# utiasASRL/mm_masking

Hardware: AMD Instinct MI355X
Metric: scan-pairs/s (mask-CNN + 10-iter dICP fwd+bwd) (higher is better)
Workload: dtype bf16; 1 GPU; BASELINE configs[2]: train_icp_weights step fwd+bwd, batch=32 per GPU, 10 dICP iters, point-to-plane Huber, dim=2; 400x3360 polar radar -> GO-CFAR + peaks + polar->Cartesian 640x640 -> U-Net (hand-written NHWC bf16 MFMA kernels, fp32 masters) -> dICP (fp32 points, fp64 normal equations) -> rot+trans+mask_pts loss -> Adam; batch_per_gpu=32, global_batch=32, scan_pts_pad=5120, map_pts=20000, map_pts_pad=20480, icp_iters=10, parallelism=dp1, scene_density=survey (SURVEY.md 8d: 3 500-5 000 valid scan points of 5 120)

## Files before the change

### mm_masking_amd/csrc/mmk_icp.hip

```cpp
#include <math.h>
#include <stdio.h>
#include <stdlib.h>

#include <algorithm>
#include <type_traits>

#include "mmk_common.h"

namespace {

constexpr int NN_THREADS = 256;
constexpr int NN_TILE = 1024;
constexpr float NN_PAD = 3.0e18f;
constexpr int ACC_THREADS = 256;
constexpr int PART_ROWS = 32;

__host__ __device__ constexpr int nacc(int dim) { return dim == 2 ? 9 : 27; }
__host__ __device__ constexpr int npose(int dim) { return dim == 2 ? 6 : 12; }

template <int DIM>
__device__ __forceinline__ void transform_point(const float *T, const float s[3], float p[DIM])
{
    if constexpr (DIM == 2) {
        p[0] = (T[0] * s[0] + T[1] * s[1]) + T[3];
        p[1] = (T[4] * s[0] + T[5] * s[1]) + T[7];
    } else {
        p[0] = ((T[0] * s[0] + T[1] * s[1]) + T[2] * s[2]) + T[3];
        p[1] = ((T[4] * s[0] + T[5] * s[1]) + T[6] * s[2]) + T[7];
        p[2] = ((T[8] * s[0] + T[9] * s[1]) + T[10] * s[2]) + T[11];
    }
}

template <int DIM>
__device__ __forceinline__ float nn_dist(float tx, float ty, float tz, const float p[DIM])
{
    float dx = tx - p[0];
    float dy = ty - p[1];
    float d = __builtin_fmaf(dy, dy, dx * dx);
    if constexpr (DIM == 3) {
        float dz = tz - p[2];
        d = __builtin_fmaf(dz, dz, d);
    }
    return d;
}

__global__ void pack_target_kernel(const float *__restrict__ tgt, int M, int cols, int dim, int Mpad,
                                   float *__restrict__ out, float *__restrict__ dec, int dec_stride)
{
    int j = blockIdx.x * blockDim.x + threadIdx.x;
    int b = blockIdx.y;
    if (j >= Mpad) return;
    for (int c = 0; c < dim; ++c) {
        float v = NN_PAD;
        if (j < M) v = tgt[((size_t)b * M + j) * cols + c];
        out[((size_t)b * dim + c) * Mpad + j] = v;
        if (dec != nullptr && j % dec_stride == 0) dec[((size_t)b * dim + c) * (Mpad / dec_stride) + j / dec_stride] = v;
    }
}

constexpr int PF_CH = 32;

__global__ __launch_bounds__(NN_THREADS) void src_zero_scan_kernel(const float *__restrict__ src, int N, int pts, int nsb,
                                                                  int32_t *__restrict__ allzero, int32_t *__restrict__ zrep)
{
    const int sb = blockIdx.x, b = blockIdx.y;
    int first = N;
    int nonzero = 0;
    for (int q = threadIdx.x; q < pts; q += blockDim.x) {
        const int i = sb * pts + q;
        if (i < N) {
            const float *sp = src + ((size_t)b * N + i) * 3;
            const bool z = sp[0] == 0.f && sp[1] == 0.f && sp[2] == 0.f;
            nonzero |= z ? 0 : 1;
            if (z && i < first) first = i;
        }
    }
    const int any = __syncthreads_or(nonzero);
#pragma unroll
    for (int off = 32; off > 0; off >>= 1) first = min(first, __shfl_down(first, off, 64));
    if ((threadIdx.x & 63) == 0 && first < N) atomicMin(&zrep[b], first);
    if (threadIdx.x == 0) allzero[(size_t)b * nsb + sb] = any ? 0 : 1;
}

__global__ void src_units_kernel(const int32_t *__restrict__ allzero, const int32_t *__restrict__ zrep, int B, int nsb, int pts,
                                 int cap, int32_t *__restrict__ ulist, int32_t *__restrict__ ucnt)
{
    const int c = threadIdx.x;
    int n = 0;
    if (c < 8)
        for (int b = c; b < B; b += 8)
            for (int sb = 0; sb < nsb; ++sb)
                if (!(allzero[(size_t)b * nsb + sb] != 0 && zrep[b] < sb * pts)) ulist[(size_t)c * cap + n++] = (b << 12) | sb;
    if (c < 8) ucnt[c] = n;
    int mx = n;
#pragma unroll
    for (int off = 4; off > 0; off >>= 1) mx = max(mx, __shfl_down(mx, off, 64));
    if (c == 0) ucnt[8] = mx;
}

typedef __attribute__((ext_vector_type(8))) __bf16 nn_bf16x8;
typedef __attribute__((ext_vector_type(16))) float nn_f32x16;
constexpr int NNM_GROUPS = 4;
constexpr int NNM_PTS = NN_THREADS / 64 * NNM_GROUPS * 32;

__device__ __forceinline__ nn_f32x16 mfma_32x32x16_bf16_c0(nn_bf16x8 a, nn_bf16x8 b)
{
    const nn_f32x16 z = {0.f, 0.f, 0.f, 0.f, 0.f, 0.f, 0.f, 0.f, 0.f, 0.f, 0.f, 0.f, 0.f, 0.f, 0.f, 0.f};
    return __builtin_amdgcn_mfma_f32_32x32x16_bf16(a, b, z, 0, 0, 0);
}
__device__ __forceinline__ void split3(float x, __bf16 &x1, __bf16 &x2, __bf16 &x3)
{
    x1 = (__bf16)x;
    const float r = x - (float)x1;
    x2 = (__bf16)r;
    x3 = (__bf16)(r - (float)x2);
}

template <int DIM>
__global__ __launch_bounds__(NN_THREADS, DIM == 2 ? 4 : 3) void nn_mfma_kernel(
    const float *__restrict__ src, const float *__restrict__ tgtp,
    const float *__restrict__ Tk, const int32_t *__restrict__ active, const int32_t *__restrict__ prev_idx,
    const int32_t *__restrict__ ulist, const int32_t *__restrict__ ucnt, int ucap, int B,
    int N, int Mpad, int nsb, int ntu, int tiles_per_unit, int total_units, float kappa,
    unsigned long long *__restrict__ packed)
{
    static_assert((DIM == 2 || DIM == 3) && NNM_GROUPS == 4, "the matrix-core filter: 16 (dim 2) or 2 x 16 (dim 3) k-slots, 4 point groups per wave");
    constexpr int KS = DIM == 2 ? 1 : 2;
    constexpr int TT = NN_TILE / KS;
    constexpr int NCH = TT / 32;
    constexpr int TPT = TT / NN_THREADS;
    __shared__ __attribute__((aligned(16))) uint4 frag[KS][NCH][64];
    __shared__ __attribute__((aligned(16))) float lt[DIM][TT];
    const int tid = threadIdx.x, lane = tid & 63, wv = tid >> 6;
    const int col = lane & 31, half = lane >> 5;
    const int ntiles = Mpad / NN_TILE;
    if (ulist != nullptr) total_units = ucnt[8] * ntu * 8;
    const float kp1 = 1.0f + kappa;

    for (int u = blockIdx.x; u < total_units; u += gridDim.x) {
        const int xcd = u & 7;
        int rest = u >> 3;
        const int tu = rest % ntu;
        rest /= ntu;
        int sb, b;
        if (ulist != nullptr) {
            if (rest >= ucnt[xcd]) continue;
            const int code = ulist[(size_t)xcd * ucap + rest];
            sb = code & 0xfff;
            b = code >> 12;
        } else {
            sb = rest % nsb;
            b = (rest / nsb) * 8 + xcd;
        }
        if (b >= B) continue;
        if (active != nullptr && active[b] == 0) continue;

        float T[16];
#pragma unroll
        for (int i = 0; i < 16; ++i) T[i] = Tk[(size_t)b * 16 + i];
        const float *tb = tgtp + (size_t)b * DIM * Mpad;

        float px[NNM_GROUPS], py[NNM_GROUPS], pz[NNM_GROUPS], c2[NNM_GROUPS], brun[NNM_GROUPS], thr[NNM_GROUPS], dseed[NNM_GROUPS];
        int jseed[NNM_GROUPS];
        nn_bf16x8 bfr[KS][NNM_GROUPS];
        unsigned w[NNM_GROUPS];
#pragma unroll
        for (int g = 0; g < NNM_GROUPS; ++g) {
            const int i = sb * NNM_PTS + wv * (NNM_GROUPS * 32) + g * 32 + col;
            float s0 = 0.f, s1 = 0.f, s2 = 0.f;
            if (i < N) {
                const float *sp = src + ((size_t)b * N + i) * 3;
                s0 = sp[0];
                s1 = sp[1];
                s2 = sp[2];
            }
            const float s[3] = {s0, s1, s2};
            float tp[DIM];
            transform_point<DIM>(T, s, tp);
            px[g] = tp[0];
            py[g] = tp[1];
            pz[g] = DIM == 3 ? tp[DIM - 1] : 0.f;
            float pn = tp[0] * tp[0] + tp[1] * tp[1];
            if constexpr (DIM == 3) pn += tp[DIM - 1] * tp[DIM - 1];
            c2[g] = 2.0f * kappa * pn + 1e-30f;
            const float ax = -2.0f * tp[0], ay = -2.0f * tp[1], az = -2.0f * pz[g];
            __bf16 ax1, ax2, ax3, ay1, ay2, ay3;
            split3(ax, ax1, ax2, ax3);
            split3(ay, ay1, ay2, ay3);
            const __bf16 one = (__bf16)1.0f, zero = (__bf16)0.0f;
            const nn_bf16x8 lo = {ax1, ax1, ax2, ax1, ax2, ax3, ay1, ay1};
            if constexpr (DIM == 2) {
                const nn_bf16x8 hi = {ay2, ay1, ay2, ay3, one, one, one, zero};
                bfr[0][g] = half ? hi : lo;
            } else {
                __bf16 az1, az2, az3;
                split3(az, az1, az2, az3);
                const nn_bf16x8 hi = {ay2, ay1, ay2, ay3, az1, az1, az2, az1};
                const nn_bf16x8 lo1 = {az2, az3, one, one, one, zero, zero, zero};
                const nn_bf16x8 hi1 = {zero, zero, zero, zero, zero, zero, zero, zero};
                bfr[0][g] = half ? hi : lo;
                bfr[KS - 1][g] = half ? hi1 : lo1;
// ... 64 lines not shown
                    *reinterpret_cast<float2 *>(&lt[0][lpos]) = vx;
                    *reinterpret_cast<float2 *>(&lt[1][lpos]) = vy;
                    *reinterpret_cast<float2 *>(&lt[DIM - 1][lpos]) = vz;
                    xs[0] = vx.x; xs[TPT - 1] = vx.y;
                    ys[0] = vy.x; ys[TPT - 1] = vy.y;
                    zs[0] = vz.x; zs[TPT - 1] = vz.y;
                }
                uint4 *fr = &frag[0][ch][p4];
#pragma unroll
                for (int r = 0; r < TPT; ++r) {
                    float n = __builtin_fmaf(ys[r], ys[r], xs[r] * xs[r]);
                    if constexpr (DIM == 3) n = __builtin_fmaf(zs[r], zs[r], n);
                    __bf16 x1, x2, x3, y1, y2, y3, n1, n2, n3;
                    split3(xs[r], x1, x2, x3);
                    split3(ys[r], y1, y2, y3);
                    split3(n, n1, n2, n3);
                    const nn_bf16x8 lo = {x1, x2, x1, x3, x2, x1, y1, y2};
                    fr[r] = __builtin_bit_cast(uint4, lo);
                    if constexpr (DIM == 2) {
                        const nn_bf16x8 hi = {y1, y3, y2, y1, n1, n2, n3, (__bf16)0.0f};
                        fr[32 + r] = __builtin_bit_cast(uint4, hi);
                    } else {
                        __bf16 z1, z2, z3;
                        split3(zs[r], z1, z2, z3);
                        const __bf16 zero = (__bf16)0.0f;
                        const nn_bf16x8 hi = {y1, y3, y2, y1, z1, z2, z1, z3};
                        const nn_bf16x8 lo1 = {z2, z1, n1, n2, n3, zero, zero, zero};
                        const nn_bf16x8 hi1 = {zero, zero, zero, zero, zero, zero, zero, zero};
                        fr[32 + r] = __builtin_bit_cast(uint4, hi);
                        uint4 *fr1 = &frag[KS - 1][ch][p4];
                        fr1[r] = __builtin_bit_cast(uint4, lo1);
                        fr1[32 + r] = __builtin_bit_cast(uint4, hi1);
                    }
                }
            }
            __syncthreads();
#pragma unroll
            for (int g = 0; g < NNM_GROUPS; ++g) w[g] = 0u;
            auto reduce = [&](const nn_f32x16 &acc, int g, bool refresh) {
                auto m3 = [](float a, float b, float c) { return __builtin_fminf(__builtin_fminf(a, b), c); };
                const float m0 = m3(thr[g], acc[0], acc[1]), m1 = m3(acc[2], acc[3], acc[4]), m2 = m3(acc[5], acc[6], acc[7]);
                const float m4 = m3(acc[8], acc[9], acc[10]), m5 = m3(acc[11], acc[12], acc[13]);
                const float n0 = m3(m0, m1, m2), n1 = m3(m4, m5, acc[14]);
                const float t = m3(n0, n1, acc[15]);
                w[g] = __builtin_amdgcn_alignbit(w[g], __float_as_uint(t - thr[g]), 31);
                brun[g] = __builtin_fminf(brun[g], t);
                if (refresh) thr[g] = __builtin_fmaf(brun[g], kp1, c2[g]);
            };
            uint4 af_next[KS];
#pragma unroll
            for (int k = 0; k < KS; ++k) af_next[k] = frag[k][0][lane];
#pragma unroll 2
            for (int c = 0; c < NCH; ++c) {
                nn_bf16x8 af[KS];
#pragma unroll
                for (int k = 0; k < KS; ++k) {
                    af[k] = __builtin_bit_cast(nn_bf16x8, af_next[k]);
                    af_next[k] = frag[k][(c + 1) & (NCH - 1)][lane];
                }
                const bool refresh = (c & 1) != 0;
#pragma unroll
                for (int h2 = 0; h2 < NNM_GROUPS; h2 += 2) {
                    nn_f32x16 acc0 = mfma_32x32x16_bf16_c0(af[0], bfr[0][h2]);
                    nn_f32x16 acc1 = mfma_32x32x16_bf16_c0(af[0], bfr[0][h2 + 1]);
                    if constexpr (KS == 2) {
                        acc0 = __builtin_amdgcn_mfma_f32_32x32x16_bf16(af[KS - 1], bfr[KS - 1][h2], acc0, 0, 0, 0);
                        acc1 = __builtin_amdgcn_mfma_f32_32x32x16_bf16(af[KS - 1], bfr[KS - 1][h2 + 1], acc1, 0, 0, 0);
                    }
                    reduce(acc0, h2, refresh);
                    reduce(acc1, h2 + 1, refresh);
                }
            }
            unsigned wo[2];
            {
                unsigned wf[NNM_GROUPS];
#pragma unroll
                for (int g = 0; g < NNM_GROUPS; ++g) {
                    const unsigned wg = NCH == 32 ? w[g] : (w[g] << (32 - NCH));
                    wf[g] = wg | (unsigned)__shfl_xor((int)wg, 32, 64);
                }
                wo[0] = half ? wf[2] : wf[0];
                wo[1] = half ? wf[3] : wf[1];
            }
            while (__any((wo[0] | wo[1]) != 0u)) {
                if ((wo[0] | wo[1]) != 0u) {
                    const bool second = wo[0] == 0u;
                    const unsigned ww = second ? wo[1] : wo[0];
                    const int c = __clz((int)ww);
                    const unsigned rest = ww & ~(0x80000000u >> c);
                    wo[0] = second ? wo[0] : rest;
                    wo[1] = second ? rest : wo[1];
                    float pq[DIM];
                    pq[0] = second ? pox[1] : pox[0];
                    pq[1] = second ? poy[1] : poy[0];
                    if constexpr (DIM == 3) pq[DIM - 1] = second ? poz[1] : poz[0];
                    const int o0 = c * 32;
                    float best = INFINITY;
                    int bj = 0;
#pragma unroll
                    for (int h = 0; h < 8; ++h) {
                        const float4 vx = *reinterpret_cast<const float4 *>(&lt[0][o0 + h * 4]);
                        const float4 vy = *reinterpret_cast<const float4 *>(&lt[1][o0 + h * 4]);
                        float4 vz = make_float4(0.f, 0.f, 0.f, 0.f);
                        if constexpr (DIM == 3) vz = *reinterpret_cast<const float4 *>(&lt[DIM - 1][o0 + h * 4]);
                        const float d0 = nn_dist<DIM>(vx.x, vy.x, vz.x, pq), d1 = nn_dist<DIM>(vx.y, vy.y, vz.y, pq);
                        const float d2 = nn_dist<DIM>(vx.z, vy.z, vz.z, pq), d3 = nn_dist<DIM>(vx.w, vy.w, vz.w, pq);
                        if (d0 < best) { best = d0; bj = h * 4 + 0; }
                        if (d1 < best) { best = d1; bj = h * 4 + 1; }
                        if (d2 < best) { best = d2; bj = h * 4 + 2; }
                        if (d3 < best) { best = d3; bj = h * 4 + 3; }
                    }
                    const int jn = t * TT + o0 + bj;
                    if (!second && best < cur[0]) { cur[0] = best; jj[0] = jn; }
                    if (second && best < cur[1]) { cur[1] = best; jj[1] = jn; }
                }
            }
        }

#pragma unroll
        for (int q = 0; q < 2; ++q) {
            const int i = pidx[q];
            if (i >= N) continue;
            if (!(cur[q] < INFINITY) && tu != 0) continue;
            const bool holds_seed = jso[q] >= t0 * NN_TILE && jso[q] < t1 * NN_TILE;
            if (jso[q] >= 0 && !holds_seed && !(cur[q] <= dso[q])) continue;
            if (holds_seed && !(cur[q] <= dso[q])) {
                cur[q] = dso[q];
                jj[q] = jso[q];
            }
            const unsigned long long key =
                ((unsigned long long)__float_as_uint(cur[q]) << 32) | (unsigned long long)(unsigned)jj[q];
            atomicMin(&packed[(size_t)b * N + i], key);
        }
    }
}

constexpr int NN_COARSE_STRIDE = 64, NN_COARSE_TILE = 1024, NN_COARSE_THREADS = 256;
typedef __attribute__((ext_vector_type(2))) float nn_f32x2;
template <int DIM>
__global__ __launch_bounds__(NN_COARSE_THREADS) void nn_coarse_seed_kernel(const float *__restrict__ src, const float *__restrict__ tgtp,
                                                             const float *__restrict__ Tk, const int32_t *__restrict__ active,
                                                             const int32_t *__restrict__ allzero, const int32_t *__restrict__ zrep,
                                                             int nn_pts, int nsb, int N, int Mpad, const float *__restrict__ dec,
                                                             int32_t *__restrict__ seed)
{
    __shared__ __attribute__((aligned(16))) float st[DIM][NN_COARSE_TILE];
    const int b = blockIdx.y;
    if (active != nullptr && active[b] == 0) return;
    if (allzero != nullptr) {
        const int sb = (blockIdx.x * NN_COARSE_THREADS) / nn_pts;
        if (sb < nsb && allzero[(size_t)b * nsb + sb] != 0 && zrep[b] < sb * nn_pts) return;
    }
    const int i = blockIdx.x * NN_COARSE_THREADS + threadIdx.x;
    float T[16];
#pragma unroll
    for (int q = 0; q < 16; ++q) T[q] = Tk[(size_t)b * 16 + q];
    float p[DIM] = {};
    if (i < N) {
        const float *sp = src + ((size_t)b * N + i) * 3;
        const float s[3] = {sp[0], sp[1], sp[2]};
        transform_point<DIM>(T, s, p);
    }
    const float *tb = tgtp + (size_t)b * DIM * Mpad;
    const int ns = Mpad / NN_COARSE_STRIDE;
    unsigned best = 0x7f800000u;
    int best_tile = 0;
    const nn_f32x2 npx = {-p[0], -p[0]}, npy = {-p[1], -p[1]}, npz = {-p[DIM - 1], -p[DIM - 1]};
    for (int s0 = 0; s0 < ns; s0 += NN_COARSE_TILE) {
        __syncthreads();
        for (int q = threadIdx.x; q < NN_COARSE_TILE; q += NN_COARSE_THREADS) {
            const int sidx = s0 + q;
#pragma unroll
            for (int c = 0; c < DIM; ++c)
                st[c][q] = sidx >= ns ? 3e18f
                                      : (dec != nullptr ? dec[((size_t)b * DIM + c) * ns + sidx] : tb[(size_t)c * Mpad + (size_t)sidx * NN_COARSE_STRIDE]);
        }
        __syncthreads();
        const int cnt = min(NN_COARSE_TILE, ns - s0);
        unsigned tb_best = 0x7f800000u;
        for (int q = 0; q < cnt; q += 4) {
            const float4 vx = *reinterpret_cast<const float4 *>(&st[0][q]);
            const float4 vy = *reinterpret_cast<const float4 *>(&st[1][q]);
            const nn_f32x2 dx0 = nn_f32x2{vx.x, vx.y} + npx, dx1 = nn_f32x2{vx.z, vx.w} + npx;
            const nn_f32x2 dy0 = nn_f32x2{vy.x, vy.y} + npy, dy1 = nn_f32x2{vy.z, vy.w} + npy;
            nn_f32x2 d0 = dx0 * dx0, d1 = dx1 * dx1;
            d0 = __builtin_elementwise_fma(dy0, dy0, d0);
            d1 = __builtin_elementwise_fma(dy1, dy1, d1);
            if (DIM == 3) {
                const float4 vz = *reinterpret_cast<const float4 *>(&st[DIM - 1][q]);
                const nn_f32x2 dz0 = nn_f32x2{vz.x, vz.y} + npz, dz1 = nn_f32x2{vz.z, vz.w} + npz;
                d0 = __builtin_elementwise_fma(dz0, dz0, d0);
                d1 = __builtin_elementwise_fma(dz1, dz1, d1);
            }
            const unsigned k0 = (__float_as_uint(d0[0]) & 0xfffffc00u) | (unsigned)q;
            const unsigned k1 = (__float_as_uint(d0[1]) & 0xfffffc00u) | (unsigned)(q + 1);
            const unsigned k2 = (__float_as_uint(d1[0]) & 0xfffffc00u) | (unsigned)(q + 2);
            const unsigned k3 = (__float_as_uint(d1[1]) & 0xfffffc00u) | (unsigned)(q + 3);
// ... 1418 lines not shown
    unsigned long long *ab = acc + (size_t)b * M * L;
    const int j0 = __shfl(j, __ffsll(vmask) - 1, 64);
    if (__ballot(valid && j != j0) == 0ull) {
#pragma unroll
        for (int off = 32; off >= L; off >>= 1) v += __shfl_xor(v, off, 64);
        if ((threadIdx.x & 63) < L && v != 0) atomicAdd(&ab[(size_t)j0 * L + c], (unsigned long long)v);
    } else if (v != 0) {
        atomicAdd(&ab[(size_t)j * L + c], (unsigned long long)v);
    }
}

__global__ void icp_bwd_target_final_kernel(const unsigned long long *__restrict__ acc, const unsigned *__restrict__ pmax,
                                            int cnt_bits, int M, int dim, int C, int L, int cols, float *__restrict__ gtgt)
{
    const int j = blockIdx.x * blockDim.x + threadIdx.x, b = blockIdx.y;
    if (j >= M) return;
    const double scale = tgt_fixed_scale(pmax[b], cnt_bits);
    const unsigned long long *a = acc + ((size_t)b * M + j) * L;
    float *out = gtgt + ((size_t)b * M + j) * cols;
    for (int c = 0; c < cols; ++c) {
        const int e = c < dim ? c : (C > dim && c >= 3 && c < 3 + dim ? dim + (c - 3) : -1);
        float v = 0.f;
        if (e >= 0) v = scale == 0.0 ? __builtin_nanf("") : (float)((double)(long long)a[e] / scale);
        out[c] = v;
    }
}

template <class F>
auto with_bool(bool b, F &&f)
{
    return b ? f(std::true_type{}) : f(std::false_type{});
}

template <class F>
auto with_dim(int dim, F &&f)
{
    return dim == 2 ? f(std::integral_constant<int, 2>{}) : f(std::integral_constant<int, 3>{});
}

template <class F>
auto with_dim_type(int dim, int icp_type, F &&f)
{
    return with_dim(dim, [&](auto D) {
        return icp_type == MMK_ICP_PT2PT ? f(D, std::integral_constant<int, MMK_ICP_PT2PT>{})
                                         : f(D, std::integral_constant<int, MMK_ICP_PT2PL>{});
    });
}

template <class F>
auto with_bools(bool a, bool b, F &&f)
{
    return with_bool(a, [&](auto A) { return with_bool(b, [&](auto B) { return f(A, B); }); });
}

inline int acc_blocks(int N) { return (N + ACC_THREADS - 1) / ACC_THREADS; }

struct NNPlan {
    int Mpad, ntiles, nsb, ntu, tiles_per_unit, total_units, grid, P, ucap;
};

NNPlan nn_plan(int B, int N, int M, int dim)
{
    NNPlan pl;
    pl.P = 2;
    pl.Mpad = (int)mmk::align_up((size_t)M, NN_TILE);
    pl.ntiles = pl.Mpad / NN_TILE;
    pl.nsb = (N + NN_THREADS * pl.P - 1) / (NN_THREADS * pl.P);
    pl.tiles_per_unit = std::min(4, pl.ntiles);
    pl.ntu = (pl.ntiles + pl.tiles_per_unit - 1) / pl.tiles_per_unit;
    const int Bpad = (B + 7) / 8 * 8;
    pl.total_units = Bpad * pl.nsb * pl.ntu;
    pl.ucap = (Bpad / 8) * pl.nsb;
    pl.grid = std::min(pl.total_units, dim == 2 ? 1024 : 768);
    return pl;
}

struct NNProf {
    bool on = false;
    int cap = 0, n = 0;
    hipEvent_t *ev = nullptr;
};
thread_local NNProf g_prof;

int launch_nn(int dim, const float *src, const float *tgtp, const float *Tk, const int32_t *active,
              const int32_t *prev_idx, const int32_t *ulist, const int32_t *ucnt, int B, int N, const NNPlan &pl,
              unsigned long long *packed, int32_t *seed_buf, const int32_t *allzero, const int32_t *zrep, const float *dec,
              hipStream_t st)
{
    const bool rec = g_prof.on && g_prof.n < g_prof.cap;
    if (rec) MMK_CHECK_HIP(hipEventRecord(g_prof.ev[2 * g_prof.n], st));
    if (prev_idx == nullptr && seed_buf != nullptr && pl.Mpad >= 4 * NN_COARSE_STRIDE) {
        const dim3 grid((N + NN_COARSE_THREADS - 1) / NN_COARSE_THREADS, B);
        const int nn_pts = NN_THREADS * pl.P;
        with_dim(dim, [&](auto D) {
            hipLaunchKernelGGL(nn_coarse_seed_kernel<D()>, grid, dim3(NN_COARSE_THREADS), 0, st, src, tgtp, Tk, active, allzero, zrep, nn_pts,
                               pl.nsb, N, pl.Mpad, dec, seed_buf);
        });
        MMK_LAUNCH_CHECK();
        prev_idx = seed_buf;
    }
    constexpr float U = 5.9604645e-8f;
    with_dim(dim, [&](auto D) {
        hipLaunchKernelGGL((nn_mfma_kernel<D()>), dim3(pl.grid), dim3(NN_THREADS), 0, st, src, tgtp, Tk, active, prev_idx, ulist, ucnt,
                           pl.ucap, B, N, pl.Mpad, pl.nsb, pl.ntu, pl.tiles_per_unit, pl.total_units, (D() == 2 ? 360.0f : 496.0f) * U,
                           packed);
    });
    MMK_LAUNCH_CHECK();
    if (rec) {
        MMK_CHECK_HIP(hipEventRecord(g_prof.ev[2 * g_prof.n + 1], st));
        g_prof.n++;
    }
    return MMK_OK;
}

int check_params(const mmk_icp_params *p)
{
    MMK_REQUIRE(p != nullptr, "mmk_icp: params is NULL");
    MMK_REQUIRE(p->B >= 1 && p->N >= 1 && p->M >= 1, "mmk_icp: B, N, M must be >= 1 (got %d, %d, %d)", p->B, p->N, p->M);
    MMK_REQUIRE(p->dim == 2 || p->dim == 3, "mmk_icp: dim must be 2 or 3 (got %d)", p->dim);
    MMK_REQUIRE(p->tgt_cols == 3 || p->tgt_cols == 6, "mmk_icp: target must have 3 or 6 columns (got %d)", p->tgt_cols);
    MMK_REQUIRE(p->icp_type == MMK_ICP_PT2PT || p->icp_type == MMK_ICP_PT2PL, "mmk_icp: bad icp_type %d", p->icp_type);
    MMK_REQUIRE(p->icp_type != MMK_ICP_PT2PL || p->tgt_cols == 6, "mmk_icp: pt2pl needs target normals (B,M,6)");
    MMK_REQUIRE(p->loss >= MMK_LOSS_NONE && p->loss <= MMK_LOSS_WELSCH, "mmk_icp: bad loss %d", p->loss);
    MMK_REQUIRE(p->max_iter >= 1, "mmk_icp: max_iter must be >= 1");
    MMK_REQUIRE(p->loss == MMK_LOSS_NONE || p->loss_k > 0.f, "mmk_icp: loss metric must be > 0");
    MMK_REQUIRE(p->nn_method == MMK_NN_BRUTE || p->nn_method == MMK_NN_GRID, "mmk_icp: bad nn_method %d", p->nn_method);
    MMK_REQUIRE(std::isfinite(p->trim_steep) && p->trim_steep >= 0.f, "mmk_icp: trim_steep must be finite and >= 0 (got %g)",
                (double)p->trim_steep);
    return MMK_OK;
}

struct RobustArgs {
    int loss;
    float k, k2, trim2, trim_dist, trim_steep;
};

RobustArgs robust_args(const mmk_icp_params *p)
{
    return {p->loss, p->loss_k, p->loss_k * p->loss_k, p->trim_dist * p->trim_dist, p->trim_dist, p->trim_steep};
}

struct IcpWs {
    float *tgtp;
    unsigned long long *packed;
    int32_t *allzero, *zrep;
    int32_t *ulist, *ucnt;
    int32_t *seed0;
    float *tdec;
    double *partials;
    double *G0, *G1;
    double *lam;
    int32_t *status;
    int32_t *g_counts, *g_cursor, *g_starts;
    float4 *g_sorted;
    size_t bytes;
};

IcpWs carve(const mmk_icp_params *p, void *ws, size_t cap)
{
    const NNPlan pl = nn_plan(p->B, p->N, p->M, p->dim);
    const int nblk = acc_blocks(p->N);
    mmk::Arena ar(ws, cap);
    IcpWs w;
    w.tgtp = ar.take<float>((size_t)p->B * p->dim * pl.Mpad);
    w.packed = ar.take<unsigned long long>((size_t)2 * p->B * p->N);
    w.allzero = ar.take<int32_t>((size_t)p->B * pl.nsb);
    w.zrep = ar.take<int32_t>((size_t)p->B);
    w.ulist = ar.take<int32_t>((size_t)8 * pl.ucap);
    w.ucnt = ar.take<int32_t>(16);
    w.seed0 = ar.take<int32_t>((size_t)p->B * p->N);
    w.tdec = ar.take<float>((size_t)p->B * p->dim * (pl.Mpad / NN_COARSE_STRIDE));
    w.partials = ar.take<double>((size_t)p->B * nblk * 27);
    w.G0 = ar.take<double>((size_t)p->B * 16);
    w.G1 = ar.take<double>((size_t)p->B * 16);
    w.lam = ar.take<double>((size_t)p->B * 6);
    w.status = ar.take<int32_t>(16);
    w.g_counts = w.g_cursor = w.g_starts = nullptr;
    w.g_sorted = nullptr;
    if (p->nn_method == MMK_NN_GRID) {
        w.g_counts = ar.take<int32_t>((size_t)p->B * GRID_NC * 2);
        w.g_cursor = w.g_counts + (size_t)p->B * GRID_NC;
        w.g_starts = ar.take<int32_t>((size_t)p->B * (GRID_NC + 1));
        w.g_sorted = ar.take<float4>((size_t)p->B * p->M);
    }
    w.bytes = mmk::align_up(ar.off, 256);
    return w;
}

// ... 14 lines not shown
    IcpBwdWs b;
    b.w = carve(p, ws, cap);
    mmk::Arena ar(ws, cap);
    ar.off = b.w.bytes;
    if (with_target) {
        const int C = tgt_row_cols(p->dim, p->icp_type);
        b.rows = ar.take<float>((size_t)p->max_iter * p->B * p->N * std::max(soft_k, 1) * C);
        b.acc = ar.take<unsigned long long>((size_t)p->B * p->M * tgt_acc_cols(C));
        b.pmax = ar.take<unsigned>((size_t)p->B);
    }
    if (with_hyper) b.hparts = ar.take<double>((size_t)p->max_iter * p->B * acc_blocks(p->N) * 3);
    if (soft_k > 0) b.soft_keys = ar.take<unsigned long long>((size_t)p->B * p->N * soft_k);
    if (with_temp) b.tparts = ar.take<double>((size_t)p->max_iter * p->B * acc_blocks(p->N));
    b.bytes = mmk::align_up(ar.off, 256);
    return b;
}

int check_workspace(const char *who, int code, const void *ws, size_t have, size_t need)
{
    if (ws != nullptr && need <= have) return MMK_OK;
    mmk::set_error(code == MMK_ERR_ARG ? "%s: workspace too small (%zu < %zu bytes)" : "%s: workspace too small (%zu < %zu)", who, have,
                   need);
    return code;
}

struct IcpCall {
    const float *source, *target, *weight;
    int32_t *idx_hist;
    float *T_hist;
    double *delta_hist, *A_hist;
    int32_t *active_hist;
    hipStream_t st;
    const float *hyper = nullptr;
    int hstride = 0;
    const float *grad_T = nullptr;
    float *grad_weight = nullptr, *grad_T_init = nullptr;
    float *grad_source = nullptr, *grad_target = nullptr;
    float *grad_hyper = nullptr;
    int soft_k = 0;
    float soft_temp = 0.f;
    const float *temp = nullptr;
    int tstride = 0;
    float *grad_temp = nullptr;
};

int check_soft(const char *who, const mmk_icp_soft *s, int M)
{
    MMK_REQUIRE(s != nullptr, "%s: soft is NULL", who);
    MMK_REQUIRE(s->k >= 2 && s->k <= SOFT_KMAX, "%s: soft.k must be in 2..%d (got %d)", who, SOFT_KMAX, s->k);
    MMK_REQUIRE(M >= s->k, "%s: the target must have at least soft.k = %d rows (got M = %d)", who, s->k, M);
    MMK_REQUIRE(std::isfinite(s->temp) && s->temp > 0.f, "%s: soft.temp must be finite and > 0 (got %g)", who, (double)s->temp);
    return MMK_OK;
}

template <class T>
T *writable(const T *p) { return const_cast<T *>(p); }

int build_grid(const float *points, int B, int M, int cols, int dim, int32_t *counts, int32_t *cursor, int32_t *starts,
               float4 *sorted, hipStream_t st)
{
    MMK_CHECK_HIP(hipMemsetAsync(counts, 0, sizeof(int32_t) * (size_t)B * GRID_NC * 2, st));
    hipLaunchKernelGGL(grid_count_kernel, dim3((M + 255) / 256, B), dim3(256), 0, st, points, M, cols, counts);
    MMK_LAUNCH_CHECK();
    hipLaunchKernelGGL(grid_scan_kernel, dim3(B), dim3(256), 0, st, counts, starts);
    MMK_LAUNCH_CHECK();
    hipLaunchKernelGGL(grid_fill_kernel, dim3((M + 255) / 256, B), dim3(256), 0, st, points, M, cols, dim, starts, cursor, sorted);
    MMK_LAUNCH_CHECK();
    return MMK_OK;
}

template <int DIM, int TYPE>
int run_forward(const mmk_icp_params *p, const IcpCall &c, const IcpWs &w, int *iters_run, unsigned long long *soft_keys = nullptr)
{
    const int B = p->B, N = p->N, M = p->M;
    const float *const src = c.source, *const tgt = c.target;
    const hipStream_t st = c.st;
    const NNPlan pl = nn_plan(B, N, M, DIM);
    const int nblk = acc_blocks(N);
    const bool soft = c.soft_k > 0;
    SoftArgs sa{soft_keys, c.soft_k, c.soft_temp, c.temp, c.temp ? c.tstride : 0};
    const size_t idx_step = p->save_state ? (size_t)B * N * (soft ? c.soft_k : 1) : 0;
    int k_done = 0;
    const bool use_grid = p->nn_method == MMK_NN_GRID;
    const int nn_pts = NN_THREADS * pl.P;
    const bool dedup = !use_grid && pl.nsb <= 0xfff && B < (1 << 19);
    if (dedup) {
        hipLaunchKernelGGL(src_zero_scan_kernel, dim3(pl.nsb, B), dim3(NN_THREADS), 0, st, src, N, nn_pts, pl.nsb, w.allzero, w.zrep);
        MMK_LAUNCH_CHECK();
        hipLaunchKernelGGL(src_units_kernel, dim3(1), dim3(64), 0, st, w.allzero, w.zrep, B, pl.nsb, nn_pts, pl.ucap, w.ulist, w.ucnt);
        MMK_LAUNCH_CHECK();
    }
    const int32_t *az = dedup ? w.allzero : nullptr, *zr = dedup ? w.zrep : nullptr;
    if (use_grid) {
        const int rc = build_grid(tgt, B, M, p->tgt_cols, DIM, w.g_counts, w.g_cursor, w.g_starts, w.g_sorted, st);
        if (rc != MMK_OK) return rc;
    }
    const RobustArgs r = robust_args(p);
    const float *const hyper = c.hyper;
    const int hstride = hyper ? c.hstride : 0;
    for (int it = 0; it < p->max_iter; ++it) {
        const float *Tk = c.T_hist + (size_t)it * B * 16;
        const int32_t *act = c.active_hist + (size_t)it * B;
        int32_t *idx = c.idx_hist + it * idx_step;
        const int32_t *prev = (it > 0) ? c.idx_hist + (it - 1) * idx_step : nullptr;
        unsigned long long *keys = w.packed + (size_t)(it & 1) * B * N, *keys_next = w.packed + (size_t)((it + 1) & 1) * B * N;
        if (use_grid) {
            const bool rec = g_prof.on && g_prof.n < g_prof.cap;
            if (rec) MMK_CHECK_HIP(hipEventRecord(g_prof.ev[2 * g_prof.n], st));
            if (soft)
                hipLaunchKernelGGL(grid_knn_kernel<DIM>, dim3((N + KNN_THREADS - 1) / KNN_THREADS, B), dim3(KNN_THREADS), 0, st, src, Tk,
                                   act, w.g_starts, w.g_sorted, N, M, c.soft_k, soft_keys);
            else
                hipLaunchKernelGGL(grid_nn_kernel<DIM>, dim3((N + 255) / 256, B), dim3(256), 0, st, src, Tk, act, w.g_starts,
                                   w.g_sorted, N, M, tgt, p->tgt_cols, prev, keys);
            MMK_LAUNCH_CHECK();
            if (rec) {
                MMK_CHECK_HIP(hipEventRecord(g_prof.ev[2 * g_prof.n + 1], st));
                g_prof.n++;
            }
        } else {
            int rc = launch_nn(DIM, src, w.tgtp, Tk, act, prev, dedup ? w.ulist : nullptr, w.ucnt, B, N, pl, keys, w.seed0, az, zr, w.tdec, st);
            if (rc != MMK_OK) return rc;
        }
        const int hcheck = hyper && it == 0 ? 1 : 0;
        sa.tcheck = c.temp && it == 0 ? 1 : 0;
        with_bools(hyper != nullptr, soft, [&](auto HP, auto SOFT) {
            if constexpr (!(HP() && SOFT()))
                hipLaunchKernelGGL((icp_accumulate_kernel<DIM, TYPE, HP(), SOFT()>), dim3(nblk, B), dim3(ACC_THREADS), 0, st, src, tgt,
                                   p->tgt_cols, c.weight, Tk, act, keys, keys_next, az, zr, nn_pts, pl.nsb, idx, N, M, r.loss, r.k, r.k2,
                                   r.trim2, r.trim_dist, r.trim_steep, w.partials, w.status, hyper, hstride, hcheck, sa);
        });
        MMK_LAUNCH_CHECK();
        hipLaunchKernelGGL(icp_solve_kernel<DIM>, dim3(B), dim3(64), 0, st, w.partials, nblk, Tk,
                           c.T_hist + (size_t)(it + 1) * B * 16, c.delta_hist + (size_t)it * B * 6,
                           c.A_hist + (size_t)it * B * 36, act, c.active_hist + (size_t)(it + 1) * B, p->tolerance);
        MMK_LAUNCH_CHECK();
        k_done = it + 1;
        if (p->check_every > 0 && (k_done % p->check_every) == 0 && k_done < p->max_iter) {
            static thread_local int32_t host_act[1 << 16];
            MMK_REQUIRE(B <= (1 << 16), "mmk_icp_forward: check_every needs B <= 65536");
            MMK_CHECK_HIP(hipMemcpyAsync(host_act, c.active_hist + (size_t)k_done * B, sizeof(int32_t) * B,
                                         hipMemcpyDeviceToHost, st));
            MMK_CHECK_HIP(hipStreamSynchronize(st));
            bool any = false;
            for (int b = 0; b < B; ++b) any = any || host_act[b] != 0;
            if (!any) break;
        }
    }
    for (int it = k_done; it < p->max_iter; ++it) {
        MMK_CHECK_HIP(hipMemcpyAsync(c.T_hist + (size_t)(it + 1) * B * 16, c.T_hist + (size_t)it * B * 16,
                                     sizeof(float) * B * 16, hipMemcpyDeviceToDevice, st));
        MMK_CHECK_HIP(hipMemsetAsync(c.active_hist + (size_t)(it + 1) * B, 0, sizeof(int32_t) * B, st));
        MMK_CHECK_HIP(hipMemsetAsync(c.delta_hist + (size_t)it * B * 6, 0, sizeof(double) * B * 6, st));
    }
    if (iters_run) *iters_run = k_done;
    return MMK_OK;
}

template <int DIM, int TYPE>
int run_backward(const mmk_icp_params *p, const IcpCall &c, const IcpBwdWs &bw)
{
    const int B = p->B, N = p->N, M = p->M;
    const IcpWs &w = bw.w;
    const hipStream_t st = c.st;
    const int nblk = acc_blocks(N);
    const RobustArgs r = robust_args(p);
    constexpr int C = tgt_row_cols(DIM, TYPE), L = tgt_acc_cols(C);
    float *const gw = c.grad_weight, *const gsrc = c.grad_source, *const gtgt = c.grad_target;
    MMK_CHECK_HIP(hipMemsetAsync(gw, 0, sizeof(float) * (size_t)B * N, st));
    if (gsrc) MMK_CHECK_HIP(hipMemsetAsync(gsrc, 0, sizeof(float) * (size_t)B * N * 3, st));
    if (gtgt) {
        MMK_CHECK_HIP(hipMemsetAsync(bw.acc, 0, sizeof(unsigned long long) * (size_t)B * M * L, st));
        MMK_CHECK_HIP(hipMemsetAsync(bw.pmax, 0, sizeof(unsigned) * (size_t)B, st));
    }
    hipLaunchKernelGGL(f32_to_f64_kernel, dim3((B * 16 + 255) / 256), dim3(256), 0, st, c.grad_T, w.G0, B * 16);
    MMK_LAUNCH_CHECK();
    double *Gin = w.G0, *Gout = w.G1;
    int nparts = 0;
    const bool pts = gsrc || gtgt, hp = bw.hparts != nullptr;
    const bool soft = c.soft_k > 0;
    const int rpp = soft ? c.soft_k : 1;
    SoftArgs sa{nullptr, c.soft_k, c.soft_temp, c.temp, c.temp ? c.tstride : 0};
    for (int it = p->max_iter - 1; it >= 0; --it) {
        const float *Tk = c.T_hist + (size_t)it * B * 16;
        const int32_t *act = c.active_hist + (size_t)it * B;
        const double *delta = c.delta_hist + (size_t)it * B * 6;
        hipLaunchKernelGGL(icp_bwd_pair_kernel<DIM>, dim3(B), dim3(64), 0, st, Gin, w.partials, nparts, Tk, delta,
                           c.A_hist + (size_t)it * B * 36, act, Gout, w.lam);
        MMK_LAUNCH_CHECK();
        float *rows = gtgt ? bw.rows + (size_t)it * B * N * rpp * C : nullptr;
        double *hparts = hp ? bw.hparts + (size_t)it * B * nblk * 3 : nullptr;
        const int32_t *idx = c.idx_hist + (size_t)it * B * N * rpp;
        sa.tparts = bw.tparts ? bw.tparts + (size_t)it * B * nblk : nullptr;
        with_bools(pts, hp, [&](auto PTS, auto HP) {
            with_bool(soft, [&](auto SOFT) {
                if constexpr (!(HP() && SOFT()))
                    hipLaunchKernelGGL((icp_bwd_point_kernel<DIM, TYPE, PTS(), HP(), SOFT()>), dim3(nblk, B), dim3(ACC_THREADS), 0, st,
                                       c.source, c.target, p->tgt_cols, c.weight, Tk, act, idx, w.lam, delta, N, M, r.loss, r.k, r.k2,
                                       r.trim2, r.trim_dist, r.trim_steep, gw, w.partials, gsrc, rows, bw.pmax, c.hyper, c.hstride,
                                       hparts, sa);
            });
        });
        MMK_LAUNCH_CHECK();
        nparts = nblk;
        std::swap(Gin, Gout);
    }
    if (c.grad_T_init) {
        hipLaunchKernelGGL(bwd_final_kernel<DIM>, dim3(B), dim3(64), 0, st, Gin, w.partials, nparts, c.grad_T_init);
        MMK_LAUNCH_CHECK();
    }
    if (c.grad_hyper) {
        hipLaunchKernelGGL(icp_bwd_hyper_final_kernel<3>, dim3(B), dim3(64), 0, st, bw.hparts, p->max_iter, B, nblk, c.grad_hyper);
        MMK_LAUNCH_CHECK();
    }
    if (c.grad_temp) {
        hipLaunchKernelGGL(icp_bwd_hyper_final_kernel<1>, dim3(B), dim3(64), 0, st, bw.tparts, p->max_iter, B, nblk, c.grad_temp);
        MMK_LAUNCH_CHECK();
    }
    if (gtgt) {
        int cnt_bits = 0;
        const int NR = N * rpp;
        while (((uint64_t)1 << cnt_bits) < (uint64_t)p->max_iter * (uint64_t)NR) ++cnt_bits;
        const unsigned gx = (unsigned)(((size_t)NR * L + ACC_THREADS - 1) / ACC_THREADS);
        hipLaunchKernelGGL(icp_bwd_target_scatter_kernel<C>, dim3(gx, B, p->max_iter), dim3(ACC_THREADS), 0, st, bw.rows, c.idx_hist,
                           c.active_hist, bw.pmax, B, NR, M, cnt_bits, bw.acc);
        MMK_LAUNCH_CHECK();
        hipLaunchKernelGGL(icp_bwd_target_final_kernel, dim3((M + 255) / 256, B), dim3(256), 0, st, bw.acc, bw.pmax, cnt_bits, M, DIM, C,
                           L, p->tgt_cols, gtgt);
        MMK_LAUNCH_CHECK();
    }
    return MMK_OK;
}

}

extern "C" int32_t mmk_nn_padded_m(int32_t M) { return (int32_t)mmk::align_up((size_t)std::max(M, 1), NN_TILE); }

extern "C" int mmk_pack_target(const float *target, int32_t B, int32_t M, int32_t tgt_cols, int32_t dim,
                               float *target_planar, void *stream)
{
    MMK_REQUIRE(target && target_planar, "mmk_pack_target: NULL pointer");
    MMK_REQUIRE(B >= 1 && M >= 1, "mmk_pack_target: B, M must be >= 1");
    MMK_REQUIRE((dim == 2 || dim == 3) && tgt_cols >= dim, "mmk_pack_target: dim must be 2|3 and <= tgt_cols");
    const int Mpad = mmk_nn_padded_m(M);
    hipLaunchKernelGGL(pack_target_kernel, dim3(Mpad / 256, B), dim3(256), 0, (hipStream_t)stream, target, M, tgt_cols,
                       dim, Mpad, target_planar, static_cast<float *>(nullptr), 1);
    MMK_LAUNCH_CHECK();
    return MMK_OK;
}

extern "C" size_t mmk_nn_workspace_bytes(int32_t B, int32_t N, int32_t M, int32_t dim)
{
    (void)dim;
    if (B < 1 || N < 1 || M < 1) return 0;
    return mmk::align_up((size_t)B * N * sizeof(unsigned long long), 256) + mmk::align_up((size_t)B * N * sizeof(int32_t), 256) + 512;
}

extern "C" int mmk_nn_search(const float *source, const float *target_planar, const float *T, int32_t B, int32_t N,
                             int32_t M, int32_t dim, int32_t *idx, float *d2, void *workspace, size_t workspace_bytes,
                             void *stream)
{
    MMK_REQUIRE(source && target_planar && T && idx && d2, "mmk_nn_search: NULL pointer");
    MMK_REQUIRE(B >= 1 && N >= 1 && M >= 1, "mmk_nn_search: B, N, M must be >= 1");
    MMK_REQUIRE(dim == 2 || dim == 3, "mmk_nn_search: dim must be 2 or 3");
    const NNPlan pl = nn_plan(B, N, M, dim);
    mmk::Arena ar(workspace, workspace_bytes);
    unsigned long long *packed = ar.take<unsigned long long>((size_t)B * N);
    int32_t *seed0 = ar.take<int32_t>((size_t)B * N);
    if (!ar.ok() || workspace == nullptr) {
        mmk::set_error("mmk_nn_search: workspace too small (%zu < %zu)", workspace_bytes, ar.off);
        return MMK_ERR_WORKSPACE;
    }
    hipStream_t st = (hipStream_t)stream;
    MMK_CHECK_HIP(hipMemsetAsync(packed, 0xFF, sizeof(unsigned long long) * (size_t)B * N, st));
    int rc = launch_nn(dim, source, target_planar, T, nullptr, nullptr, nullptr, nullptr, B, N, pl, packed, seed0, nullptr, nullptr, nullptr, st);
    if (rc != MMK_OK) return rc;
    hipLaunchKernelGGL(nn_unpack_kernel, dim3((B * N + 255) / 256), dim3(256), 0, st, packed, B * N, idx, d2);
    MMK_LAUNCH_CHECK();
    return MMK_OK;
}

namespace {

struct KnnWs {
    int32_t *counts, *cursor, *starts;
    float4 *sorted;
    size_t bytes;
};

KnnWs knn_carve(int32_t B, int32_t M, void *workspace, size_t workspace_bytes)
{
    mmk::Arena ar(workspace, workspace_bytes);
    KnnWs w;
    w.counts = ar.take<int32_t>((size_t)B * GRID_NC * 2);
    w.cursor = w.counts + (size_t)B * GRID_NC;
    w.starts = ar.take<int32_t>((size_t)B * (GRID_NC + 1));
    w.sorted = ar.take<float4>((size_t)B * M);
    w.bytes = mmk::align_up(ar.off, 256);
    return w;
}

template <int DIM, int KC>
void knn_launch(const float *points, int B, int M, int cols, int k, float max_radius, float pad_val, const float *viewpoint,
                const KnnWs &w, float *normals, float *curvature, int32_t *count, int32_t *nbr_idx, hipStream_t st)
{
    hipLaunchKernelGGL((knn_normals_kernel<DIM, KC>), dim3((M + KNN_THREADS - 1) / KNN_THREADS, B), dim3(KNN_THREADS), 0, st, points,
                       M, cols, k, max_radius, pad_val, viewpoint, w.starts, w.sorted, normals, curvature, count, nbr_idx);
}

}

extern "C" size_t mmk_knn_normals_workspace_bytes(int32_t B, int32_t M)
{
    if (B < 1 || M < 1) return 0;
    return knn_carve(B, M, nullptr, 0).bytes;
}

extern "C" int mmk_knn_normals(const float *points, int32_t B, int32_t M, int32_t cols, int32_t dim, int32_t k, float max_radius,
                               float pad_val, const float *viewpoint, float *normals, float *curvature, int32_t *count,
                               int32_t *nbr_idx, void *workspace, size_t workspace_bytes, void *stream)
{
    MMK_REQUIRE(points && normals, "mmk_knn_normals: NULL pointer");
    MMK_REQUIRE(B >= 1 && M >= 1 && B <= 65535, "mmk_knn_normals: B must be in 1..65535 and M >= 1 (got %d, %d)", B, M);
    MMK_REQUIRE((dim == 2 || dim == 3) && cols >= dim, "mmk_knn_normals: dim must be 2|3 and <= cols");
    MMK_REQUIRE(k >= 3 && k <= 32, "mmk_knn_normals: k must be in 3..32 (got %d)", k);
    const KnnWs w = knn_carve(B, M, workspace, workspace_bytes);
    int rc = check_workspace("mmk_knn_normals", MMK_ERR_WORKSPACE, workspace, workspace_bytes, w.bytes);
    if (rc != MMK_OK) return rc;
    hipStream_t st = (hipStream_t)stream;
    rc = build_grid(points, B, M, cols, dim, w.counts, w.cursor, w.starts, w.sorted, st);
    if (rc != MMK_OK) return rc;
#define KNN_GO(KC) knn_launch<D(), KC>(points, B, M, cols, k, max_radius, pad_val, viewpoint, w, normals, curvature, count, nbr_idx, st)
    with_dim(dim, [&](auto D) {
        if (k <= 8) KNN_GO(8);
        else if (k <= 16) KNN_GO(16);
        else KNN_GO(32);
    });
#undef KNN_GO
    MMK_LAUNCH_CHECK();
    return MMK_OK;
}

extern "C" int mmk_nn_profile_begin(int32_t capacity)
{
    MMK_REQUIRE(capacity >= 1 && capacity <= (1 << 20), "mmk_nn_profile_begin: bad capacity %d", capacity);
    if (g_prof.cap < capacity) {
        for (int i = 0; i < 2 * g_prof.cap; ++i) (void)hipEventDestroy(g_prof.ev[i]);
        delete[] g_prof.ev;
        g_prof.ev = new hipEvent_t[2 * (size_t)capacity];
        g_prof.cap = 0;
        for (int i = 0; i < 2 * capacity; ++i) MMK_CHECK_HIP(hipEventCreate(&g_prof.ev[i]));
        g_prof.cap = capacity;
    }
    g_prof.n = 0;
    g_prof.on = true;
    return MMK_OK;
}

// ... 365 lines not shown
```

Baseline: 3454 pairs/s.

## Switch sparse NN candidate refinement to wave-cooperative per-chunk evaluation

In the MFMA nearest-neighbour kernel, the per-lane serial refinement of flagged 32-point chunks now runs only while at least a threshold number of lanes still have pending chunks. The leftover sparse chunks are handled cooperatively: each pass broadcasts one lane's query point and chunk index, all 32 lanes of the half-wave compute one distance each, and DPP min-reductions plus ballots pick the minimum and its index. This targets divergence, where a few lanes with many candidate chunks keep the whole wave looping. The old path stays available through an environment variable, and the new path adds cross-lane reduction overhead with possibly different tie-breaking on equal distances.

```diff
diff --git a/mm_masking_amd/csrc/mmk_icp.hip b/mm_masking_amd/csrc/mmk_icp.hip
--- a/mm_masking_amd/csrc/mmk_icp.hip
+++ b/mm_masking_amd/csrc/mmk_icp.hip
@@ -59,6 +59,7 @@
 }
 
 constexpr int PF_CH = 32;
+constexpr int NN_DENSE_MIN = 8;
 
 __global__ __launch_bounds__(NN_THREADS) void src_zero_scan_kernel(const float *__restrict__ src, int N, int pts, int nsb,
                                                                   int32_t *__restrict__ allzero, int32_t *__restrict__ zrep)
@@ -116,7 +117,7 @@
     x3 = (__bf16)(r - (float)x2);
 }
 
-template <int DIM>
+template <int DIM, bool LEGACY>
 __global__ __launch_bounds__(NN_THREADS, DIM == 2 ? 4 : 3) void nn_mfma_kernel(
     const float *__restrict__ src, const float *__restrict__ tgtp,
     const float *__restrict__ Tk, const int32_t *__restrict__ active, const int32_t *__restrict__ prev_idx,
@@ -347,7 +348,12 @@
                 wo[0] = half ? wf[2] : wf[0];
                 wo[1] = half ? wf[3] : wf[1];
             }
-            while (__any((wo[0] | wo[1]) != 0u)) {
+            auto lane_round_due = [&]() {
+                const unsigned long long f = __ballot((wo[0] | wo[1]) != 0u);
+                return LEGACY ? f != 0ull : __popcll(f) >= NN_DENSE_MIN;
+            };
+#pragma nounroll
+            for (int round = 0; round < 2 * NCH && lane_round_due(); ++round) {
                 if ((wo[0] | wo[1]) != 0u) {
                     const bool second = wo[0] == 0u;
                     const unsigned ww = second ? wo[1] : wo[0];
@@ -378,6 +384,53 @@
                     const int jn = t * TT + o0 + bj;
                     if (!second && best < cur[0]) { cur[0] = best; jj[0] = jn; }
                     if (second && best < cur[1]) { cur[1] = best; jj[1] = jn; }
+                }
+            }
+            if constexpr (!LEGACY) {
+                auto rowmin = [](unsigned v) {
+                    auto step = [](unsigned x, auto CTRL) {
+                        return min(x, (unsigned)__builtin_amdgcn_update_dpp(0, (int)x, CTRL(), 0xf, 0xf, true));
+                    };
+                    v = step(v, std::integral_constant<int, 0xB1>{});
+                    v = step(v, std::integral_constant<int, 0x4E>{});
+                    v = step(v, std::integral_constant<int, 0x141>{});
+                    return step(v, std::integral_constant<int, 0x140>{});
+                };
+#pragma unroll
+                for (int q = 0; q < 2; ++q) {
+#pragma nounroll
+                    for (int pass = 0; pass < NCH * 32; ++pass) {
+                        const bool has = wo[q] != 0u;
+                        const unsigned long long left = __ballot(has);
+                        if (left == 0ull) break;
+                        const int olo = __builtin_ctz((unsigned)left | 0x80000000u);
+                        const int ohi = 32 + __builtin_ctz((unsigned)(left >> 32) | 0x80000000u);
+                        const int own4 = half ? ohi << 2 : olo << 2;
+                        const int c = __clz((int)wo[q]);
+                        auto bcast = [&](int v) { return __builtin_amdgcn_ds_bpermute(own4, v); };
+                        float pq[DIM];
+                        pq[0] = __int_as_float(bcast(__float_as_int(pox[q])));
+                        pq[1] = __int_as_float(bcast(__float_as_int(poy[q])));
+                        if constexpr (DIM == 3) pq[DIM - 1] = __int_as_float(bcast(__float_as_int(poz[q])));
+                        const int ci = bcast(c) & (NCH - 1);
+                        const int o = ci * 32 + col;
+                        const float d = nn_dist<DIM>(lt[0][o], lt[1][o], DIM == 3 ? lt[DIM - 1][o] : 0.f, pq);
+                        const unsigned du = __float_as_uint(__builtin_fminf(d, INFINITY));
+                        unsigned m = rowmin(du);
+                        m = min(m, (unsigned)__builtin_amdgcn_update_dpp((int)m, (int)m, 0x142, 0xa, 0xf, false));
+                        const unsigned mlo = (unsigned)__builtin_amdgcn_readlane((int)m, 31), mhi = (unsigned)__builtin_amdgcn_readlane((int)m, 63);
+                        const unsigned eq_lo = (unsigned)__ballot(du == mlo), eq_hi = (unsigned)(__ballot(du == mhi) >> 32);
+                        const int wlo = __builtin_ctz(eq_lo | 0x80000000u), whi = __builtin_ctz(eq_hi | 0x80000000u);
+                        m = half ? mhi : mlo;
+                        if (has && (lane << 2) == own4) {
+                            wo[q] &= ~(0x80000000u >> c);
+                            const float best = __uint_as_float(m);
+                            if (best < cur[q]) {
+                                cur[q] = best;
+                                jj[q] = t * TT + c * 32 + (half ? whi : wlo);
+                            }
+                        }
+                    }
                 }
             }
         }
@@ -1962,10 +2015,16 @@
 };
 thread_local NNProf g_prof;
 
+bool nn_legacy()
+{
+    const char *e = getenv("MMK_NN_LEGACY");
+    return e != nullptr && e[0] == '1';
+}
+
 int launch_nn(int dim, const float *src, const float *tgtp, const float *Tk, const int32_t *active,
               const int32_t *prev_idx, const int32_t *ulist, const int32_t *ucnt, int B, int N, const NNPlan &pl,
               unsigned long long *packed, int32_t *seed_buf, const int32_t *allzero, const int32_t *zrep, const float *dec,
-              hipStream_t st)
+              bool legacy, hipStream_t st)
 {
     const bool rec = g_prof.on && g_prof.n < g_prof.cap;
     if (rec) MMK_CHECK_HIP(hipEventRecord(g_prof.ev[2 * g_prof.n], st));
@@ -1981,9 +2040,11 @@
     }
     constexpr float U = 5.9604645e-8f;
     with_dim(dim, [&](auto D) {
-        hipLaunchKernelGGL((nn_mfma_kernel<D()>), dim3(pl.grid), dim3(NN_THREADS), 0, st, src, tgtp, Tk, active, prev_idx, ulist, ucnt,
-                           pl.ucap, B, N, pl.Mpad, pl.nsb, pl.ntu, pl.tiles_per_unit, pl.total_units, (D() == 2 ? 360.0f : 496.0f) * U,
-                           packed);
+        with_bool(legacy, [&](auto LEGACY) {
+            hipLaunchKernelGGL((nn_mfma_kernel<D(), LEGACY()>), dim3(pl.grid), dim3(NN_THREADS), 0, st, src, tgtp, Tk, active, prev_idx,
+                               ulist, ucnt, pl.ucap, B, N, pl.Mpad, pl.nsb, pl.ntu, pl.tiles_per_unit, pl.total_units,
+                               (D() == 2 ? 360.0f : 496.0f) * U, packed);
+        });
     });
     MMK_LAUNCH_CHECK();
     if (rec) {
@@ -2164,6 +2225,7 @@
     const size_t idx_step = p->save_state ? (size_t)B * N * (soft ? c.soft_k : 1) : 0;
     int k_done = 0;
     const bool use_grid = p->nn_method == MMK_NN_GRID;
+    const bool legacy_nn = nn_legacy();
     const int nn_pts = NN_THREADS * pl.P;
     const bool dedup = !use_grid && pl.nsb <= 0xfff && B < (1 << 19);
     if (dedup) {
@@ -2201,7 +2263,8 @@
                 g_prof.n++;
             }
         } else {
-            int rc = launch_nn(DIM, src, w.tgtp, Tk, act, prev, dedup ? w.ulist : nullptr, w.ucnt, B, N, pl, keys, w.seed0, az, zr, w.tdec, st);
+            int rc = launch_nn(DIM, src, w.tgtp, Tk, act, prev, dedup ? w.ulist : nullptr, w.ucnt, B, N, pl, keys, w.seed0, az, zr, w.tdec,
+                               legacy_nn, st);
             if (rc != MMK_OK) return rc;
         }
         const int hcheck = hyper && it == 0 ? 1 : 0;
@@ -2355,7 +2418,8 @@
     }
     hipStream_t st = (hipStream_t)stream;
     MMK_CHECK_HIP(hipMemsetAsync(packed, 0xFF, sizeof(unsigned long long) * (size_t)B * N, st));
-    int rc = launch_nn(dim, source, target_planar, T, nullptr, nullptr, nullptr, nullptr, B, N, pl, packed, seed0, nullptr, nullptr, nullptr, st);
+    int rc = launch_nn(dim, source, target_planar, T, nullptr, nullptr, nullptr, nullptr, B, N, pl, packed, seed0, nullptr, nullptr, nullptr,
+                       nn_legacy(), st);
     if (rc != MMK_OK) return rc;
     hipLaunchKernelGGL(nn_unpack_kernel, dim3((B * N + 255) / 256), dim3(256), 0, st, packed, B * N, idx, d2);
     MMK_LAUNCH_CHECK();
```

New measurement: 3439 pairs/s. No clear change (-0.4%).
